# barry-mir/mixing-style-transfer

Measured on AMD Instinct MI355X. Metric: triplets/sec (10 s @ 44.1 kHz, 4-stem, bs=24), higher is better.
Workload: dtype f32

## Files before the change

### mixing-style-transfer_amd/csrc/encoder.hip

```cpp
#include "common.h"

#include <cmath>
#include <type_traits>
#include <vector>

namespace {

typedef float f32x4 __attribute__((ext_vector_type(4)));
constexpr int kConvThreads = 512;
constexpr int kConvWaves = 8;

struct FilmParams {
  const float* feats;
  const float *w0t, *b0, *w3t, *b3, *hwt, *hb;
  const float *s1, *t1, *s2, *t2;
  float* film;
  float2* aff1;
  float2* aff2;
  int Fd, H, nsub;
  float* h2;
  int B;
};

constexpr int kFilmCT = 8;
// ... 677 lines not shown
  int nsaddr[4] = {-1, -1, -1, -1};

  auto prefetch_setup = [&](int q, const RTile& t) __attribute__((always_inline)) {
    const int chunk = q % NCH;
    const float* src = p.in + (size_t)t.clip * p.in_clipstride + (size_t)t.band * p.in_bandoff + (size_t)(4 * chunk) * p.in_cstride;
    const float* wsrc = p.wfrag + ((size_t)t.band * NCH + chunk) * WBP;
    nrsrc = __builtin_amdgcn_make_buffer_rsrc(const_cast<float*>(src), 0, (unsigned)(4 * p.in_cstride) * 4u, 0x00020000);
    nwrsrc = __builtin_amdgcn_make_buffer_rsrc(const_cast<float*>(wsrc), 0, (unsigned)WBP * 4u, 0x00020000);
    if (chunk == 0) {
      const bool fold = t.kind == 2;
      const int row0 = (t.kind == 1 ? 4 : 0) - 3, col0 = 16 * t.blk - 3;
      const int rbase = max(row0, 0), cbase = max(col0, 0);
      nsoff = (unsigned)(rbase * p.in_cols + cbase) * 4u;
      int ln = lane;
      asm volatile("" : "+v"(ln));
#pragma unroll
      for (int j = 0; j < 4; ++j) {
        const int e = ln + 64 * j;
        const int r = fold ? e >> 4 : e / PC, c = fold ? e & 15 : e % PC;
        const bool in_patch = fold ? (r < R::FR && c < R::FC) : r < R::PR;
        const int rin = row0 + r, cin = col0 + c;
        const bool ok = t.valid && in_patch && rin >= 0 && rin < p.in_rows && cin >= 0 && cin < p.in_cols;
        nvoff[j] = ok ? (unsigned)((rin - rbase) * p.in_cols + (cin - cbase)) * 4u : 0x80000000u;
        nsaddr[j] = in_patch ? r * PC + c : -1;
      }
    }
  };
  auto prefetch_piece = [&](int i) __attribute__((always_inline)) {
    if (i < NPFK) {
      pf[i] = __builtin_bit_cast(float, __builtin_amdgcn_raw_buffer_load_b32(nrsrc, nvoff[i & 3], nsoff + (unsigned)((i >> 2) * p.in_cstride) * 4u, 0));
    } else if (i < NPIECE) {
      wreg[i - NPFK] = __builtin_bit_cast(f32x4, __builtin_amdgcn_raw_buffer_load_b128(nwrsrc, (unsigned)tid * 16u, (unsigned)(kConvThreads * (i - NPFK)) * 16u, 0));
    }
  };

  f32x4 acc[MT][NT];
  RTile cur{}, nxt{};
  nxt = decode(0);
  if (nq > 0) {
    prefetch_setup(0, nxt);
#pragma unroll
    for (int i = 0; i < NPIECE; ++i) prefetch_piece(i);
  }
#ifdef MST_TRACE
  long long trc[5] = {0, 0, 0, 0, 0};
  const long long trc_start = clock64();
#endif
  for (int q = 0; q < nq; ++q) {
    float* wb = wbuf + (q & 1) * WBP;
#ifdef MST_TRACE
    const long long tq0 = clock64();
#endif
#pragma unroll
    for (int i = 0; i < NWF; ++i) reinterpret_cast<f32x4*>(wb)[tid + kConvThreads * i] = wreg[i];
#pragma unroll
    for (int i = 0; i < NPFK; ++i)
      if (nsaddr[i & 3] >= 0) pbuf[(i >> 2) * CP + nsaddr[i & 3]] = pf[i];
#ifdef MST_TRACE
    asm volatile("s_waitcnt lgkmcnt(0)" ::: "memory");
    const long long tq1 = clock64();
#endif
    __syncthreads();
#ifdef MST_TRACE
    const long long tq2 = clock64();
    trc[0] += tq1 - tq0, trc[1] += tq2 - tq1, trc[4] += 1;
#endif
    cur = nxt;
    if ((q + 1) % NCH == 0) nxt = decode(q + 1);
    prefetch_setup(q + 1, nxt);
    const int chunk = q % NCH;
    if (chunk == 0) {
      ap = cur.kind == 2 ? ap_fold : ap_pair;
#pragma unroll
      for (int t = 0; t < MT; ++t)
#pragma unroll
        for (int n = 0; n < NT; ++n) acc[t][n] = f32x4{0.f, 0.f, 0.f, 0.f};
    }
    {
      float a[2][MT], b[2][NT];
#pragma unroll
      for (int t = 0; t < MT; ++t) a[0][t] = ap[t * PC];
#pragma unroll
      for (int n = 0; n < NT; ++n) b[0][n] = wb[n * 64 + lane];
      auto taps = [&](auto LO_, auto HI_, auto MASK_) __attribute__((always_inline)) {
        constexpr int LO = decltype(LO_)::value, HI = decltype(HI_)::value, MASK = decltype(MASK_)::value;
#pragma unroll
        for (int tap = LO; tap < HI; ++tap) {
          const int cu = tap & 1, nx = cu ^ 1;
          const int off = ((tap + 1) / 7) * PC + ((tap + 1) % 7);
#pragma unroll
          for (int i = 0; i < MT * NT; ++i) {
            const int t = i / NT, n = i % NT;
            if (!((MASK >> t) & 1)) acc[t][n] = __builtin_amdgcn_mfma_f32_16x16x4f32(a[cu][t], b[cu][n], acc[t][n], 0, 0, 0);
            if (tap + 1 < 49) {
              if (i < NT) b[nx][i] = wb[((tap + 1) * NT + i) * 64 + lane];
              else if (i < MT + NT) a[nx][i - NT] = ap[(i - NT) * PC + off];
            }
            if (i >= MT + NT && i - (MT + NT) < PPT) prefetch_piece(tap * PPT + (i - (MT + NT)));
            __builtin_amdgcn_sched_barrier(0);
          }
        }
      };
      using std::integral_constant;
      using I0 = integral_constant<int, 0>;
      using I7 = integral_constant<int, 7>;
      using I14 = integral_constant<int, 14>;
      using I21 = integral_constant<int, 21>;
      using I42 = integral_constant<int, 42>;
      using I49 = integral_constant<int, 49>;
      if (cur.kind == 0) {
        taps(I0{}, I7{}, integral_constant<int, 0b0111>{});
        taps(I7{}, I14{}, integral_constant<int, 0b0011>{});
        taps(I14{}, I21{}, integral_constant<int, 0b0001>{});
      } else {
        taps(I0{}, I21{}, I0{});
      }
      taps(I21{}, I42{}, I0{});
      if (cur.kind == 1) taps(I42{}, I49{}, integral_constant<int, 0b1000>{});
      else taps(I42{}, I49{}, I0{});
    }
#ifdef MST_TRACE
    trc[2] += clock64() - tq2;
#endif
    if (chunk == NCH - 1 && cur.valid) {
      const int j = lane & 15, g = lane >> 4;
      const float2* aff = p.aff + ((size_t)cur.clip * p.nsub + cur.band) * C::COUT;
      const int pr = cur.kind == 2 ? g >> 1 : cur.kind;
      const int pc = 4 * cur.blk + (cur.kind == 2 ? g & 1 : g);
#pragma unroll
      for (int n = 0; n < NT; ++n) {
        const int ch = n * 16 + j;
        const float2 ac = aff[ch];
        float m = 0.f;
#pragma unroll
        for (int t = 0; t < MT; ++t)
#pragma unroll
          for (int r = 0; r < 4; ++r) m = fmaxf(m, fmaf(acc[t][n][r], ac.x, ac.y));
        if (pc < p.out_cols)
          p.out[(((size_t)cur.clip * p.nsub + cur.band) * C::COUT + ch) * p.out_rows * p.out_cols + (size_t)pr * p.out_cols + pc] = m;
      }
    }
  }
#ifdef MST_TRACE
  if (lane == 0 && p.yraw) {
    float* o = p.yraw + (blockIdx.x * kConvWaves + wave) * 8;
    for (int i = 0; i < 5; ++i) o[i] = (float)trc[i];
    o[5] = (float)(clock64() - trc_start);
  }
#endif
}

template <int SUB>
constexpr size_t kConv1ResidentLds = (size_t)(2 * 49 * CC<1, SUB>::NT * 64 + kConvWaves * 8 * CC<1, SUB>::PR * CC<1, SUB>::PC) * sizeof(float);
template <int SUB, int MODE = 0, int LAY = 0>
__global__ __launch_bounds__(kConvThreads) void conv1_resident_kernel(const ConvParams p) {
  using C = CC<1, SUB>;
  constexpr int MT = C::MT, NT = C::NT, PR = C::PR, PC = C::PC;
  static_assert(C::RL == 64, "resident conv1 expects one loader row per instruction");
  static_assert(LAY == 0 || PR == 8, "the channel-minor loader maps lane bits 1..3 to the 8 patch rows");
  constexpr int WCH = 49 * NT * 64;
  constexpr int WBP = ConvGeom<1, SUB>::WBP;
  constexpr int CHS = PR * PC;
  constexpr int PATCH = 8 * CHS;
  constexpr int NPF = LAY == 0 ? 8 * PR : (PC + 3) / 4;
  extern __shared__ __attribute__((aligned(16))) float smem[];
  const int tid = threadIdx.x, lane = tid & 63;
  const int wave = __builtin_amdgcn_readfirstlane(tid >> 6);
  float* wres = smem;
  float* pbuf = smem + 2 * WCH + wave * PATCH;
  constexpr bool DYN = MODE == 0;
  constexpr int kTickets = 16;
  __shared__ unsigned tickets[kTickets];
#ifdef MST_TRACE
  long long trc[5] = {0, 0, 0, 0, 0};
  const long long trc_start = clock64();
#endif

  const int G = gridDim.x;
  const int wg = mst::xcd_remap(blockIdx.x, G);
  const int total_sets = (p.clip_major ? (p.B + p.clip_major - 1) / p.clip_major : 1) * p.nsub * p.sets_per_band;
  const int s_begin = (int)((long long)wg * total_sets / G), s_end = (int)((long long)(wg + 1) * total_sets / G);
  const int tpb = p.tiles_r * p.tiles_c;

  auto decode = [&](int s) __attribute__((always_inline)) {
    Tile t;
    int ti;
    if (p.clip_major) {
      const int ngrp = (p.B + p.clip_major - 1) / p.clip_major;
      const int gb = min(s / p.sets_per_band, ngrp * p.nsub - 1);
      const int idx = (s - gb * p.sets_per_band) * kConvWaves + wave;
      const int grp = gb / p.nsub, c0 = grp * p.clip_major;
      t.band = gb - grp * p.nsub;
      t.valid = (s < s_end) && idx < min(p.clip_major, p.B - c0) * tpb;
      const int cl = t.valid ? idx / tpb : 0;
      t.clip = c0 + cl;
      ti = t.valid ? idx - cl * tpb : 0;
    } else {
      t.band = min(s / p.sets_per_band, p.nsub - 1);
      const int idx = (s - t.band * p.sets_per_band) * kConvWaves + wave;
      t.valid = (s < s_end) && idx < p.B * tpb;
      t.clip = t.valid ? idx / tpb : 0;
      ti = t.valid ? idx - t.clip * tpb : 0;
    }
    t.tc = ti / p.tiles_r;
    t.tr = ti - t.tc * p.tiles_r;
    return t;
  };

  const int kq = lane >> 4, ai = lane & 15, ag = ai >> 2, areg = ai & 3;
  int abase[MT];
#pragma unroll
  for (int t = 0; t < MT; ++t) {
    const int e = 4 * t + areg, wv = e / C::WIN, pos = e % C::WIN;
    abase[t] = kq * CHS + (pos / 5) * PC + 5 * (C::WPG * ag + wv) + pos % 5;
  }

  typename std::conditional<LAY == 0, float, f32x4>::type pf[NPF];
  unsigned long long rowmask = 0;
  bool col_ok = false;
  int coff = 0, nrow0 = 0, nvalid = 0;
  const float* nsrc = p.in;
  bool nfast = false;
  __amdgpu_buffer_rsrc_t nrsrc = __builtin_amdgcn_make_buffer_rsrc(const_cast<float*>(p.in), 0, 0, 0x00020000);
  unsigned nsoff = 0, nvoff = 0;
  static_assert(WBP - WCH >= 4, "the chunk pitch leaves at least 16 zero bytes behind the weights");
  const float* const zero16 = p.wfrag + WCH;
  const int lr = (lane >> 1) & 7, lhalf = lane & 1, lfq = lane >> 4;
  const unsigned frame_bytes = (unsigned)p.cm_mels * 32u;
  auto prefetch_setup = [&](const Tile& t) __attribute__((always_inline)) {
    nrow0 = C::TROWS * t.tr - 3;
    nvalid = t.valid;
    rowmask = 0;
    if constexpr (LAY == 0) {
      const int col0 = C::TCOLS * t.tc - 3, cin = col0 + lane;
      nsrc = p.in + (size_t)t.clip * p.in_clipstride + (size_t)t.band * p.in_bandoff;
      col_ok = lane < PC && cin >= 0 && cin < p.in_cols;
      coff = min(max(cin, 0), p.in_cols - 1);
    } else {
      const int rin = nrow0 + lr, rc = min(max(rin, 0), p.in_rows - 1);
      nsrc = p.in + (size_t)t.clip * p.in_clipstride;
      col_ok = nvalid && rin == rc;
      coff = ((t.band * p.cm_overlap + rc) * 8 + 4 * lhalf) * 4;
      nrow0 = C::TCOLS * t.tc - 3 + lfq;
      if constexpr (DYN) {
        const int f0 = C::TCOLS * t.tc - 3;
        nfast = nvalid && f0 >= 0 && f0 + 4 * NPF + 3 < p.in_cols;
        nrsrc = __builtin_amdgcn_make_buffer_rsrc(const_cast<float*>(nsrc), 0, (unsigned)p.in_cols * frame_bytes, 0x00020000);
        nsoff = (unsigned)max(f0, 0) * frame_bytes;
        nvoff = col_ok ? (unsigned)coff + (unsigned)lfq * frame_bytes : 0x80000000u;
      }
    }
  };
  auto prefetch_piece = [&](int i) __attribute__((always_inline)) {
    if (i < NPF) {
      if constexpr (LAY == 0) {
        const int cc = i / PR, r = i % PR;
        const int rin = nrow0 + r;
        const int rc = min(max(rin, 0), p.in_rows - 1);
        if (nvalid && rin == rc) rowmask |= 1ull << i;
        const float* rowp = nsrc + (size_t)cc * p.in_cstride + (size_t)rc * p.in_cols;
        if constexpr (DYN) pf[i] = (nvalid && rin == rc && col_ok) ? rowp[coff] : *zero16;
        else pf[i] = rowp[coff];
      } else {
        const int fin = nrow0 + 4 * i, fc = min(max(fin, 0), p.in_cols - 1);
        if (col_ok && fin == fc) rowmask |= 1ull << i;
        if (DYN && nfast) {
          pf[i] = __builtin_bit_cast(f32x4, __builtin_amdgcn_raw_buffer_load_b128(nrsrc, nvoff, nsoff + (unsigned)(4 * i) * frame_bytes, 0));
        } else {
          const unsigned boff = (unsigned)fc * frame_bytes + (unsigned)coff;
          const char* src = reinterpret_cast<const char*>(nsrc) + boff;
          if constexpr (DYN) src = (col_ok && fin == fc) ? src : reinterpret_cast<const char*>(zero16);
          pf[i] = *reinterpret_cast<const f32x4*>(src);
        }
      }
    }
  };
  auto prefetch_step = [&](int ks) __attribute__((always_inline)) {
    if constexpr (LAY == 0) prefetch_piece(ks);
    else if (ks % 8 == 0) prefetch_piece(ks / 8);
  };

  f32x4 acc[MT][NT];
  double st[NT][2];
#pragma unroll
  for (int n = 0; n < NT; ++n) st[n][0] = st[n][1] = 0.0;
  int cur_band = -1;
  const int spb = p.sets_per_band;
  const int gb0 = s_begin / spb, nseg = s_end > s_begin ? (s_end - 1) / spb - gb0 + 1 : 0;
  int dseg = 0, dlo = 0, dhi = 0, dgb = 0, nxt_seg = 0;
  auto seg_range = [&](int k) __attribute__((always_inline)) {
    dgb = gb0 + k;
    const int cm = p.clip_major ? p.clip_major : p.B, grp = p.clip_major ? dgb / p.nsub : 0;
    dlo = max(s_begin - dgb * spb, 0) * kConvWaves;
    dhi = min((min(s_end, (dgb + 1) * spb) - dgb * spb) * kConvWaves, min(cm, p.B - grp * cm) * tpb);
  };
  unsigned tkv = 0;
  auto ticket_issue = [&]() __attribute__((always_inline)) {
    tkv = 0;
    if (dseg < nseg && lane == 0)
      tkv = __hip_atomic_fetch_add(&tickets[dseg % kTickets], 1u, __ATOMIC_RELAXED, __HIP_MEMORY_SCOPE_WORKGROUP);
  };
  auto ticket_take = [&]() __attribute__((always_inline)) {
    Tile t{};
    while (dseg < nseg) {
      const int idx = dlo + (int)__builtin_amdgcn_readfirstlane(tkv);
      if (idx < dhi) {
        const int grp = p.clip_major ? dgb / p.nsub : 0;
        const int cl = idx / tpb, ti = idx - cl * tpb;
        t.valid = 1;
        t.band = dgb - grp * p.nsub;
        t.clip = grp * p.clip_major + cl;
        t.tc = ti / p.tiles_r;
        t.tr = ti - t.tc * p.tiles_r;
        return t;
      }
      if (++dseg < nseg) seg_range(dseg);
      ticket_issue();
    }
    return t;
  };
  Tile cur{}, nxt{};
  if constexpr (DYN) {
    if (tid < kTickets) tickets[tid] = 0;
    __syncthreads();
    if (nseg > 0) seg_range(0);
    ticket_issue();
    nxt = ticket_take();
    nxt_seg = dseg;
  } else {
    nxt = decode(s_begin);
  }
  prefetch_setup(nxt);
#pragma unroll
  for (int i = 0; i < NPF; ++i) prefetch_piece(i);

  auto mask_piece = [&](int i) __attribute__((always_inline)) {
    if constexpr (LAY == 0) {
      pf[i] = (((rowmask >> i) & 1ull) && col_ok) ? pf[i] : 0.f;
    } else {
      const bool ok = (rowmask >> i) & 1ull;
#pragma unroll
      for (int k = 0; k < 4; ++k) pf[i][k] = ok ? pf[i][k] : 0.f;
    }
  };
  auto stage_ = [&](auto MASKED_) __attribute__((always_inline)) {
    constexpr bool MASKED = decltype(MASKED_)::value;
    if constexpr (LAY == 0) {
#pragma unroll
      for (int i = 0; i < NPF; ++i) {
        if (!MASKED) mask_piece(i);
        if (lane < PC) pbuf[i * PC + lane] = pf[i];
      }
    } else {
      float* pl = pbuf + (4 * lhalf) * CHS + lr * PC + lfq;
#pragma unroll
      for (int i = 0; i < NPF; ++i) {
        if (4 * i + 3 < PC || 4 * i + lfq < PC) {
          if (!MASKED) mask_piece(i);
#pragma unroll
          for (int k = 0; k < 4; ++k) pl[k * CHS + 4 * i] = pf[i][k];
        }
      }
    }
  };
  auto stage = [&]() __attribute__((always_inline)) { stage_(std::false_type{}); };
  auto tile_body = [&]() __attribute__((always_inline)) {
#ifdef MST_TRACE
    const long long tr0 = clock64();
#endif
#pragma unroll
    for (int t = 0; t < MT; ++t)
#pragma unroll
      for (int n = 0; n < NT; ++n) acc[t][n] = f32x4{0.f, 0.f, 0.f, 0.f};
    {
      float a[2][MT], b[2][NT];
#pragma unroll
      for (int t = 0; t < MT; ++t) a[0][t] = pbuf[abase[t]];
#pragma unroll
      for (int n = 0; n < NT; ++n) b[0][n] = wres[n * 64 + lane];
#pragma unroll
      for (int ks = 0; ks < 98; ++ks) {
        const int cu = ks & 1, nx = cu ^ 1;
        const int tap = (ks + 1) >> 1, ch = (ks + 1) & 1;
        const int off = ch * 4 * CHS + (tap / 7) * PC + (tap % 7);
#pragma unroll
        for (int i = 0; i < MT * NT; ++i) {
          const int t = i / NT, n = i % NT;
          acc[t][n] = __builtin_amdgcn_mfma_f32_16x16x4f32(a[cu][t], b[cu][n], acc[t][n], 0, 0, 0);
          if (ks + 1 < 98) {
            if (i < NT) b[nx][i] = wres[ch * WCH + (tap * NT + i) * 64 + lane];
            else if (i < MT + NT) a[nx][i - NT] = pbuf[abase[i - NT] + off];
          }
          if (i == MT + NT) prefetch_step(ks);
          __builtin_amdgcn_sched_barrier(0);
        }
      }
    }
#ifdef MST_TRACE
    const long long tr1 = clock64();
    trc[0] += tr1 - tr0, trc[4] += 1;
#endif
    if constexpr (MODE == 1) {
      const int j = lane & 15, g = lane >> 4;
      float* yb = p.yraw + ((((size_t)cur.clip * p.nsub + cur.band) * p.acc_tr + cur.tr) * p.acc_tc + cur.tc) *
                               (size_t)(NT * 64 * 4 * MT);
#pragma unroll
      for (int n = 0; n < NT; ++n) {
        const float b = p.bias[cur.band * C::COUT + n * 16 + j];
        f32x4* dst = reinterpret_cast<f32x4*>(yb) + (size_t)n * (64 * MT) + lane;
#pragma unroll
        for (int t = 0; t < MT; ++t) {
          f32x4 v = acc[t][n];
#pragma unroll
          for (int r = 0; r < 4; ++r) {
            v[r] += b;
            const int e = 4 * t + r, wv = e / C::WIN, pos = e % C::WIN;
            const int col = C::TCOLS * cur.tc + 5 * (C::WPG * g + wv) + pos % 5;
            if (col < p.raw_cols) st[n][0] += (double)v[r], st[n][1] += (double)v[r] * (double)v[r];
          }
          dst[64 * t] = v;
        }
      }
    } else
    {
      const int j = lane & 15, g = lane >> 4;
      const float2* aff = p.aff + ((size_t)cur.clip * p.nsub + cur.band) * C::COUT;
      float* orow = p.out + ((size_t)cur.clip * p.nsub + cur.band) * C::COUT * p.out_rows * p.out_cols +
                    (size_t)cur.tr * p.out_cols;
#pragma unroll
      for (int n = 0; n < NT; ++n) {
        const int ch = n * 16 + j;
        const float2 ac = aff[ch];
#pragma unroll
        for (int wv = 0; wv < C::WPG; ++wv) {
          const int pc = 4 * C::WPG * cur.tc + C::WPG * g + wv;
          if (SUB == 2 && p.pool_h == 1) {
#pragma unroll
            for (int hr = 0; hr < 2; ++hr) {
              float m = 0.f;
#pragma unroll
              for (int pos = 0; pos < 5; ++pos) {
                const int e = wv * C::WIN + 5 * hr + pos;
                m = fmaxf(m, fmaf(acc[e >> 2][n][e & 3], ac.x, ac.y));
              }
              if (pc < p.out_cols && 2 * cur.tr + hr < p.out_rows)
                orow[(size_t)ch * p.out_rows * p.out_cols + (size_t)(cur.tr + hr) * p.out_cols + pc] = m;
            }
          } else {
            float m = 0.f;
#pragma unroll
            for (int pos = 0; pos < C::WIN; ++pos) {
              const int e = wv * C::WIN + pos;
              m = fmaxf(m, fmaf(acc[e >> 2][n][e & 3], ac.x, ac.y));
            }
            if (pc < p.out_cols) orow[(size_t)ch * p.out_rows * p.out_cols + pc] = m;
          }
        }
      }
    }
#ifdef MST_TRACE
    trc[1] += clock64() - tr1;
#endif
  };
  f32x4 sav[MT][NT];
  float2 sav_ac[NT];
  Tile prev{};
#pragma unroll
  for (int t = 0; t < MT; ++t)
#pragma unroll
    for (int n = 0; n < NT; ++n) sav[t][n] = f32x4{0.f, 0.f, 0.f, 0.f};
#pragma unroll
  for (int n = 0; n < NT; ++n) sav_ac[n] = float2{0.f, 0.f};
  auto epi_part = [&](auto N_, auto WV_) __attribute__((always_inline)) {
    constexpr int n = decltype(N_)::value, wv = decltype(WV_)::value;
    const int j = lane & 15, g = lane >> 4;
    const int ch = n * 16 + j;
    float* orow = p.out + ((size_t)prev.clip * p.nsub + prev.band) * C::COUT * p.out_rows * p.out_cols + (size_t)prev.tr * p.out_cols;
    const float2 ac = sav_ac[n];
    const int pc = 4 * C::WPG * prev.tc + C::WPG * g + wv;
    if (SUB == 2 && p.pool_h == 1) {
#pragma unroll
      for (int hr = 0; hr < 2; ++hr) {
        float m = 0.f;
#pragma unroll
        for (int pos = 0; pos < 5; ++pos) {
          const int e = wv * C::WIN + 5 * hr + pos;
          m = fmaxf(m, fmaf(sav[e >> 2][n][e & 3], ac.x, ac.y));
        }
        if (prev.valid && pc < p.out_cols && 2 * prev.tr + hr < p.out_rows)
          orow[(size_t)ch * p.out_rows * p.out_cols + (size_t)(prev.tr + hr) * p.out_cols + pc] = m;
      }
    } else {
      float m = 0.f;
#pragma unroll
      for (int pos = 0; pos < C::WIN; ++pos) {
        const int e = wv * C::WIN + pos;
        m = fmaxf(m, fmaf(sav[e >> 2][n][e & 3], ac.x, ac.y));
      }
      if (prev.valid && pc < p.out_cols) orow[(size_t)ch * p.out_rows * p.out_cols + pc] = m;
    }
  };
  auto tile_dyn = [&]() __attribute__((always_inline)) {
#ifdef MST_TRACE
    const long long tr0 = clock64();
#endif
    float2 e_ac[NT];
    {
      const float2* aff = p.aff + ((size_t)cur.clip * p.nsub + cur.band) * C::COUT;
#pragma unroll
      for (int n = 0; n < NT; ++n) e_ac[n] = aff[n * 16 + (lane & 15)];
    }
    {
      constexpr int kEpi0 = 12;
      const bool skip_c = cur.tr == 0, skip_b = 2 * cur.tr + 2 >= p.in_rows;
      const int next_off = skip_b ? 0 : 5 * PC, next_w = skip_b ? 0 : 35 * NT * 64;
      float a[2][MT], b[2][NT];
#pragma unroll
      for (int t = 0; t < MT; ++t) a[0][t] = pbuf[abase[t] + 2 * PC];
#pragma unroll
      for (int n = 0; n < NT; ++n) b[0][n] = wres[(14 * NT + n) * 64 + lane];
      auto kstep = [&](auto S_) __attribute__((always_inline)) {
        constexpr int ks = decltype(S_)::value;
        constexpr int cu = ks & 1, nx = cu ^ 1;
        constexpr bool last = ks == 41 || ks == 69 || ks == 97;
        constexpr int s1 = ks + 1, l1 = s1 < 42 ? s1 : s1 < 70 ? s1 - 42 : s1 - 70;
        constexpr int row1 = (s1 < 42 ? 2 : s1 < 70 ? 5 : 0) + l1 / 14, tap1 = 7 * row1 + (l1 % 14) / 2, ch1 = l1 & 1;
        constexpr int off1 = ch1 * 4 * CHS + row1 * PC + (l1 % 14) / 2;
#pragma unroll
        for (int i = 0; i < MT * NT; ++i) {
          const int t = i / NT, n = i % NT;
          acc[t][n] = __builtin_amdgcn_mfma_f32_16x16x4f32(a[cu][t], b[cu][n], ks == 0 ? f32x4{0.f, 0.f, 0.f, 0.f} : acc[t][n], 0, 0, 0);
          if constexpr (!last) {
            if (i < NT) b[nx][i] = wres[ch1 * WCH + (tap1 * NT + i) * 64 + lane];
            else if (i < MT + NT) a[nx][i - NT] = pbuf[abase[i - NT] + off1];
          } else if constexpr (ks == 41) {
            if (i < NT) b[nx][i] = wres[next_w + i * 64 + lane];
            else if (i < MT + NT) a[nx][i - NT] = pbuf[abase[i - NT] + next_off];
          } else if constexpr (ks == 69) {
            if (i < NT) b[nx][i] = wres[i * 64 + lane];
            else if (i < MT + NT) a[nx][i - NT] = pbuf[abase[i - NT]];
          }
          if (i == MT + NT) {
            if constexpr (LAY == 0) {
              if constexpr (ks >= 8 && ks < 8 + NPF / 2) prefetch_piece(2 * (ks - 8)), prefetch_piece(2 * (ks - 8) + 1);
            } else {
              if constexpr (ks >= 8 && ks % 2 == 0 && ks / 2 - 4 < NPF) prefetch_piece(ks / 2 - 4);
            }
          }
          if (i == MT + NT + 1) {
            if constexpr (ks == 0) ticket_issue();
            if constexpr (ks == 6) {
              nxt = ticket_take();
              nxt_seg = dseg;
              prefetch_setup(nxt);
            }
            if constexpr (ks >= kEpi0 && ks < kEpi0 + 2 * NT * C::WPG && (ks - kEpi0) % 2 == 0)
              epi_part(std::integral_constant<int, (ks - kEpi0) / 2 / C::WPG>{}, std::integral_constant<int, (ks - kEpi0) / 2 % C::WPG>{});
          }
          __builtin_amdgcn_sched_barrier(0);
        }
      };
      static_assert(LAY == 0 ? 8 + NPF / 2 <= 42 : 2 * (NPF + 3) < 42, "the patch fetch must fit block A");
      static_for<42>([&](auto I) __attribute__((always_inline)) { kstep(std::integral_constant<int, decltype(I)::value>{}); });
      if (!skip_b) static_for<28>([&](auto I) __attribute__((always_inline)) { kstep(std::integral_constant<int, 42 + decltype(I)::value>{}); });
      if (!skip_c) static_for<28>([&](auto I) __attribute__((always_inline)) { kstep(std::integral_constant<int, 70 + decltype(I)::value>{}); });
    }
    {
      const float bz = wres[lane];
#pragma unroll
      for (int t = 0; t < MT; ++t)
#pragma unroll
        for (int n = 0; n < NT; ++n) sav[t][n] = __builtin_amdgcn_mfma_f32_16x16x4f32(0.f, bz, acc[t][n], 0, 0, 0);
    }
#pragma unroll
    for (int n = 0; n < NT; ++n) sav_ac[n] = e_ac[n];
    prev = cur;
#ifdef MST_TRACE
    trc[0] += clock64() - tr0, trc[4] += 1;
#endif
  };
  auto load_band = [&](int band) __attribute__((always_inline)) {
    for (int c = 0; c < 2; ++c) {
      const f32x4* src = reinterpret_cast<const f32x4*>(p.wfrag + ((size_t)band * 2 + c) * WBP);
      for (int k = tid; k < WCH / 4; k += kConvThreads) reinterpret_cast<f32x4*>(wres + c * WCH)[k] = src[k];
    }
  };
  if constexpr (DYN) {
    for (int k = 0; k < nseg; ++k) {
#ifdef MST_TRACE
      const long long tb0 = clock64();
#endif
      __syncthreads();
      load_band((gb0 + k) % p.nsub);
      if (tid == 0) tickets[(k + kTickets - 1) % kTickets] = 0;
      __syncthreads();
#ifdef MST_TRACE
      trc[3] += clock64() - tb0;
#endif
      while (nxt.valid && nxt_seg == k) {
#ifdef MST_TRACE
        const long long ts0 = clock64();
#endif
        cur = nxt;
#ifdef MST_TRACE
        asm volatile("s_waitcnt vmcnt(0)" ::: "memory");
        const long long ts1 = clock64();
        trc[1] += ts1 - ts0;
#endif
        stage_(std::true_type{});
#ifdef MST_TRACE
        asm volatile("s_waitcnt lgkmcnt(0)" ::: "memory");
        trc[2] += clock64() - ts1;
#endif
        tile_dyn();
      }
    }
    {
      static_for<NT * C::WPG>([&](auto I) __attribute__((always_inline)) {
        constexpr int q = decltype(I)::value;
        epi_part(std::integral_constant<int, q / C::WPG>{}, std::integral_constant<int, q % C::WPG>{});
      });
    }
#ifdef MST_TRACE
    if (lane == 0 && p.yraw) {
      float* o = p.yraw + (blockIdx.x * kConvWaves + wave) * 8;
      for (int i = 0; i < 5; ++i) o[i] = (float)trc[i];
      o[5] = (float)(clock64() - trc_start);
    }
#endif
  } else {
  for (int s = s_begin; s < s_end; ++s) {
    cur = nxt;
    if (cur.band != cur_band) {
      if (MODE == 1 && cur_band >= 0) flush_stats<NT, C::COUT>(st, p.stats, cur_band, lane);
      __syncthreads();
      load_band(cur.band);
      __syncthreads();
      cur_band = cur.band;
    }
    stage();
    nxt = decode(s + 1);
    prefetch_setup(nxt);
    if (!cur.valid) {
#pragma unroll
      for (int i = 0; i < NPF; ++i) prefetch_piece(i);
      continue;
    }
    tile_body();
  }
  }
  if (MODE == 1 && cur_band >= 0) flush_stats<NT, C::COUT>(st, p.stats, cur_band, lane);
}

__global__ __launch_bounds__(256) void absmax_kernel(const float* __restrict__ x, long long n_per_clip, unsigned* out) {
  const float* base = x + (size_t)blockIdx.y * n_per_clip;
  float m = 0.f;
  const long long n4 = n_per_clip >> 2;
  const float4* b4 = reinterpret_cast<const float4*>(base);
  const bool al = (reinterpret_cast<uintptr_t>(base) & 15) == 0;
  if (al) {
    for (long long i = (long long)blockIdx.x * 256 + threadIdx.x; i < n4; i += (long long)gridDim.x * 256) {
      const float4 v = b4[i];
      m = fmaxf(fmaxf(m, fmaxf(fabsf(v.x), fabsf(v.y))), fmaxf(fabsf(v.z), fabsf(v.w)));
    }
    for (long long i = (n4 << 2) + (long long)blockIdx.x * 256 + threadIdx.x; i < n_per_clip; i += (long long)gridDim.x * 256)
      m = fmaxf(m, fabsf(base[i]));
  } else {
    for (long long i = (long long)blockIdx.x * 256 + threadIdx.x; i < n_per_clip; i += (long long)gridDim.x * 256)
      m = fmaxf(m, fabsf(base[i]));
  }
  m = mst::wave_max(m);
  if ((threadIdx.x & 63) == 0) atomicMax(out + blockIdx.y, __float_as_uint(m));
}

__global__ __launch_bounds__(64) void f16_scale_kernel(const float2* __restrict__ aff1, const float* __restrict__ w1norm,
                                                        const unsigned* __restrict__ xmax_bits, float* scale, int nsub,
                                                        const float* __restrict__ bias = nullptr, float gain = 1.0f) {
  const int clip = blockIdx.x / nsub, band = blockIdx.x % nsub, c = threadIdx.x & 31;
  const float xmax = __uint_as_float(xmax_bits[clip]);
  const float2 a = aff1[((size_t)clip * nsub + band) * 32 + c];
  float bound = fmaf(fabsf(a.x), fmaf(w1norm[band * 32 + c], xmax, bias ? fabsf(bias[band * 32 + c]) : 0.f), fabsf(a.y)) * gain;
  bound = mst::wave_max(bound);
  if (threadIdx.x == 0) {
    int k = 0;
    if (bound > 0.f && bound < INFINITY) {
      int ex;
      (void)frexpf(bound, &ex);
      k = max(-60, min(60, 14 - ex));
    } else if (!(bound < INFINITY)) {
      k = -60;
    }
    scale[(size_t)blockIdx.x * 2] = ldexpf(1.0f, k);
    scale[(size_t)blockIdx.x * 2 + 1] = ldexpf(1.0f, -k);
  }
}

typedef _Float16 h16x8 __attribute__((ext_vector_type(8)));
__device__ __forceinline__ _Float16 to_f16_sat(float v) {
  return (_Float16)(__builtin_isfinite(v) ? fminf(fmaxf(v, -65504.f), 65504.f) : v);
}
__host__ inline int f16_weight_exponent(float maxabs) {
  if (!(maxabs > 0.f) || !(maxabs < INFINITY)) return 10;
  int ex;
  (void)frexpf(maxabs, &ex);
  return std::max(-100, std::min(100, 14 - ex));
}
constexpr int kF16Steps = 13;

template <int SUB>
constexpr size_t kConv1F16Lds = (size_t)(kF16Steps * CC<1, SUB>::NT * 2 * 64 + kConvWaves * 2 * CC<1, SUB>::PR * CC<1, SUB>::PC) * 16;
template <int SUB, int TERMS, int MODE = 0, int LAY = 0>
__global__ __launch_bounds__(kConvThreads) void conv1_f16x3_kernel(const ConvParams p, const h16x8* __restrict__ wfrag16,
                                                                  _Float16* __restrict__ out_hi, _Float16* __restrict__ out_lo) {
  using C = CC<1, SUB>;
  constexpr int MT = C::MT, NT = C::NT, PR = C::PR, PC = C::PC;
  static_assert(C::RL == 64, "one loader row per instruction");
  static_assert(LAY == 0 || (LAY == 2 && PR == 8), "the channel-minor loader maps lane bits 0..2 to the 8 patch rows");
  constexpr int WVEC = kF16Steps * NT * 2 * 64;
// ... 2175 lines not shown
  float* ptrs[] = {e->w1frag, e->w2frag, e->s1, e->t1, e->s2, e->t2, e->w0t, e->b0, e->w3t, e->b3, e->hwt,
                   e->hb, e->att0frag, e->att0_b, e->att2_w, e->projfrag, e->proj_b, e->c1b, e->bn1w, e->bn1b, e->c2b,
                   e->bn2w, e->bn2b, e->w2dfrag, e->att2_b, e->f16_wsc1e, e->f16_wsc2e, e->w2norm_e};
  for (float* q : ptrs) (void)hipFree(q);
  (void)hipFree(e->w1frag16), (void)hipFree(e->w1frag16e);
  (void)hipFree(e->w1norm), (void)hipFree(e->f16_winv1), (void)hipFree(e->f16_winv2);
  (void)hipFree(e->w2frag16);
  (void)hipFree(e->w2dfrag16);
  (void)hipFree(e->f16_wsc1), (void)hipFree(e->f16_wsc2), (void)hipFree(e->f16_wsc2d), (void)hipFree(e->f16_winv2d);
  (void)hipFree(e->w2norm);
  delete e;
}

int mst_encoder_set_precision(mst_encoder* e, int conv1_f16x3) {
  MST_REQUIRE(e, "mst_encoder_set_precision: NULL encoder");
  MST_REQUIRE(conv1_f16x3 == 0 || (conv1_f16x3 >= 1 && conv1_f16x3 <= 3 && (e->sub == 2 || (e->sub == 1 && e->cfg.split_size % 2 == 0))),
              "mst_encoder_set_precision: the f16 modes (1, 2, 3) need 2-row conv1 tiles (20-mel sub-bands, or an even split_size below 20)");
  e->conv1_f16x3 = conv1_f16x3;
  return MST_OK;
}

int mst_encoder_set_train_precision(mst_encoder* e, int f16_operands) {
  MST_REQUIRE(e, "mst_encoder_set_train_precision: NULL encoder");
  MST_REQUIRE(f16_operands == 0 || ((f16_operands == 1 || f16_operands == 2) && (e->sub == 2 || e->cfg.split_size % 2 == 0)),
              "mst_encoder_set_train_precision: modes 1 (f16 operands) and 2 (split precision) need 2-row conv1 tiles (20-mel sub-bands, or an even split_size below 20)");
  if (f16_operands && !e->w2dfrag16) {
    const int ns = e->cfg.n_subbands;
    bool ok = hipMalloc(&e->w2dfrag16, (size_t)ns * 8 * kF16Steps * 2 * 2 * 64 * 8 * sizeof(_Float16)) == hipSuccess;
    ok = ok && hipMalloc(&e->f16_wsc1, (size_t)ns * 32 * 4) == hipSuccess && hipMalloc(&e->f16_wsc2, (size_t)ns * 64 * 4) == hipSuccess;
    ok = ok && hipMalloc(&e->f16_wsc2d, (size_t)ns * 32 * 4) == hipSuccess && hipMalloc(&e->f16_winv2d, (size_t)ns * 32 * 4) == hipSuccess;
    ok = ok && hipMalloc(&e->w2norm, (size_t)ns * 64 * 4) == hipSuccess;
    if (!ok) return mst::fail(MST_ENOMEM, "mst_encoder_set_train_precision: out of device memory");
  }
  e->train_f16 = f16_operands;
  return MST_OK;
}

size_t mst_encoder_workspace_bytes(const mst_encoder* e, int B, int frames) {
  if (!e || B <= 0 || frames < 20) return 0;
  return ws_layout(e, B, frames).total;
}

static bool conv1_resident_geometry(const mst_encoder* e) {
  return (e->sub == 2 || (e->sub == 1 && e->cfg.split_size % 2 == 0)) && !getenv("MST_CONV1_CHUNKED");
}

int mst_encoder_layout_supported(const mst_encoder* e, int layout) {
  if (!e) return 0;
  if (layout == MST_LOGMEL_REF) return 1;
  if (e->sub > 2) return 0;
  if (layout == MST_LOGMEL_CM32) return e->conv1_f16x3 == 0 && conv1_resident_geometry(e);
  if (layout == MST_LOGMEL_CM16) return e->conv1_f16x3 != 0;
  return 0;
}

int mst_encoder_forward(const mst_encoder* e, const float* logmel, int frames, const float* feats, int B, float* emb,
                        const mst_encoder_taps* taps, void* workspace, size_t workspace_bytes, void* stream) {
  mst_logmel_in in{};
  in.layout = MST_LOGMEL_REF, in.data = logmel;
  return mst_encoder_forward_in(e, &in, frames, feats, B, emb, taps, workspace, workspace_bytes, stream);
}

int mst_encoder_forward_in(const mst_encoder* e, const mst_logmel_in* lin, int frames, const float* feats, int B, float* emb,
                           const mst_encoder_taps* taps, void* workspace, size_t workspace_bytes, void* stream) {
  MST_REQUIRE(e && lin && lin->data && feats && emb, "mst_encoder_forward: NULL argument");
  const int lay = lin->layout;
  if (const int rc = check_logmel_in("mst_encoder_forward", lin, mst_encoder_layout_supported(e, lay), e->conv1_f16x3,
                                     e->conv1_f16x3 != 3, e->conv1_f16x3 >= 2))
    return rc;
  const float* logmel = static_cast<const float*>(lin->data);
  MST_REQUIRE(B > 0 && frames >= 20, "mst_encoder_forward: need B>0 and frames>=20 (B=%d frames=%d)", B, frames);
  const WsLayout L = ws_layout(e, B, frames);
  MST_REQUIRE(L.W2 >= 1, "mst_encoder_forward: clip too short for two pooling stages (frames=%d)", frames);
  if (!workspace || workspace_bytes < L.total)
    return mst::fail(MST_ENOMEM, "mst_encoder_forward: workspace %zu B < required %zu B", workspace_bytes, L.total);
  hipStream_t st = reinterpret_cast<hipStream_t>(stream);
  char* ws = reinterpret_cast<char*>(workspace);
  const int ns = e->cfg.n_subbands;
  float* film = (taps && taps->film) ? taps->film : reinterpret_cast<float*>(ws + L.film);
  float* pool1 = (taps && taps->pool1) ? taps->pool1 : reinterpret_cast<float*>(ws + L.pool1);
  float* pool_in = (taps && taps->pool_in) ? taps->pool_in : reinterpret_cast<float*>(ws + L.pool_in);
  float2* aff1 = reinterpret_cast<float2*>(ws + L.aff1);
  float2* aff2 = reinterpret_cast<float2*>(ws + L.aff2);
  auto mark = [&](int i) {
    if (taps && taps->events[i]) (void)hipEventRecord(reinterpret_cast<hipEvent_t>(taps->events[i]), st);
  };
  mark(0);
  MST_HIP_CHECK(launch_film(film_params(e, feats, film, aff1, aff2, reinterpret_cast<float*>(ws + L.film_h2), B), st));
  mark(1);
  const int grid = e->num_cus;
  const dim3 blk(kConvThreads);
  {
    ConvParams cp{};
    cp.in = logmel, cp.wfrag = e->w1frag, cp.aff = aff1, cp.out = pool1, cp.B = B, cp.nsub = ns;
    conv1_input_geometry(cp, e, frames);
    cp.in_lo = lin->lo, cp.cm_mels = e->cfg.n_mels, cp.cm_overlap = e->cfg.overlap;
    cp.out_rows = e->H1, cp.out_cols = L.W1;
    cp.tiles_r = e->H1;
    cp.tiles_c = e->sub == 2 ? (L.W1 + 7) / 8 : (L.W1 + 15) / 16;
    const bool resident = e->sub <= 2 && !e->conv1_f16x3 && conv1_resident_geometry(e);
    if (e->sub == 1 && (e->conv1_f16x3 || resident)) {
      cp.pool_h = 1;
      cp.tiles_r = e->cfg.split_size / 2;
      cp.tiles_c = (L.W1 + 7) / 8;
    }
    cp.sets_per_band = sets_per_band(B, cp.tiles_r, cp.tiles_c);
    const int g = std::min(grid, ns * cp.sets_per_band);
    hipError_t err;
    if (e->sub > 2) {
      MST_REQUIRE(lay == MST_LOGMEL_REF && e->conv1_f16x3 == 0, "mst_encoder_forward: split_size=%d runs in the reference layout, fp32 only", e->cfg.split_size);
      err = mst::launch_lds<conv1_generic_kernel>(dim3((L.W1 + kGenCols - 1) / kGenCols, B * ns), dim3(256),
                                                  conv1_generic_lds(e->cfg.split_size), st, cp, e->sub);
    } else if (e->conv1_f16x3) {
      const bool both = e->conv1_f16x3 >= 2;
      cp.f16_winv = e->f16_winv1;
      if (both && !(taps && taps->pool1)) cp.out = nullptr;
      if (both) {
        const unsigned* xmax = lin->absmax;
        float* fsc = reinterpret_cast<float*>(ws + L.f16scale);
        if (!xmax) {
          unsigned* xm = reinterpret_cast<unsigned*>(ws + L.xmax);
          MST_HIP_CHECK(hipMemsetAsync(xm, 0, (size_t)B * sizeof(unsigned), st));
          const long long npc = (long long)8 * e->cfg.n_mels * frames;
          hipLaunchKernelGGL(absmax_kernel, dim3(64, B), dim3(256), 0, st, logmel, npc, xm);
          xmax = xm;
        }
        hipLaunchKernelGGL(f16_scale_kernel, dim3(B * ns), dim3(64), 0, st, aff1, e->w1norm, xmax, fsc, ns);
        cp.f16_scale = fsc;
      }
      const h16x8* wf = reinterpret_cast<const h16x8*>(e->w1frag16);
      _Float16* oh = both ? reinterpret_cast<_Float16*>(ws + L.pool1_h16) : nullptr;
      _Float16* ol = e->conv1_f16x3 == 2 ? reinterpret_cast<_Float16*>(ws + L.pool1_l16) : nullptr;
      if (lay == MST_LOGMEL_CM16) {
        const h16x8* wfe = reinterpret_cast<const h16x8*>(e->w1frag16e);
        if (e->conv1_f16x3 == 3) {
          cp.sets_per_band = sets_per_band(B, cp.tiles_r, cp.tiles_c, kF16eWaves<1>);
          const int g1 = std::min(grid, ns * cp.sets_per_band);
          err = mst::launch_lds<conv1_f16e_kernel<1>>(dim3(g1), dim3(kF16eWaves<1> * 64), kConv1F16eLds<1>, st, cp, wfe, oh, ol);
        }
        else err = mst::launch_lds<conv1_f16e_kernel<3>>(dim3(g), blk, kConv1F16eLds<3>, st, cp, wfe, oh, ol);
      } else if (e->conv1_f16x3 == 3) err = mst::launch_lds<conv1_f16x3_kernel<2, 1>>(dim3(g), blk, kConv1F16Lds<2>, st, cp, wf, oh, ol);
      else err = mst::launch_lds<conv1_f16x3_kernel<2, 3>>(dim3(g), blk, kConv1F16Lds<2>, st, cp, wf, oh, ol);
    } else if (resident) {
      if (!getenv("MST_CONV1_BAND_MAJOR")) {
        const char* env = getenv("MST_CONV1_CLIP_GROUP");
        cp.clip_major = std::max(1, std::min(B, env ? atoi(env) : 1));
        cp.sets_per_band = sets_per_band(cp.clip_major, cp.tiles_r, cp.tiles_c);
      }
      const int g = std::min(grid, (cp.clip_major ? (B + cp.clip_major - 1) / cp.clip_major : 1) * ns * cp.sets_per_band);
#ifdef MST_TRACE
      static ConvTrace trace;
      trace_attach(trace, cp);
#endif
      if (lay == MST_LOGMEL_CM32) err = mst::launch_lds<conv1_resident_kernel<2, 0, 1>>(dim3(g), blk, kConv1ResidentLds<2>, st, cp);
      else err = mst::launch_lds<conv1_resident_kernel<2>>(dim3(g), blk, kConv1ResidentLds<2>, st, cp);
#ifdef MST_TRACE
      trace_dump(trace, g, false);
#endif
    } else {
      err = e->sub == 2 ? launch_conv<1, 2>(cp, g, st) : launch_conv<1, 1>(cp, g, st);
    }
    if (err != hipSuccess) return mst::fail(MST_EHIP, "conv1 launch failed: %s", hipGetErrorString(err));
  }
  mark(2);
  {
    ConvParams cp{};
    cp.in = pool1, cp.wfrag = e->w2frag, cp.aff = aff2, cp.out = pool_in, cp.B = B, cp.nsub = ns;
    conv2_input_geometry(cp, e, L.W1);
    cp.out_rows = e->FD, cp.out_cols = L.W2;
    cp.tiles_r = (e->FD + 1) / 2;
    cp.tiles_c = (L.W2 + 1) / 2;
    cp.sets_per_band = sets_per_band(B, cp.tiles_r, cp.tiles_c);
    const int g = std::min(grid, ns * cp.sets_per_band);
    hipError_t err;
    if (e->conv1_f16x3 >= 2) {
      cp.f16_scale = reinterpret_cast<const float*>(ws + L.f16scale);
      cp.f16_winv = e->f16_winv2;
      const h16x8* ih = reinterpret_cast<const h16x8*>(ws + L.pool1_h16);
      const h16x8* il = reinterpret_cast<const h16x8*>(ws + L.pool1_l16);
      const h16x8* wf = reinterpret_cast<const h16x8*>(e->w2frag16);
      if (e->conv1_f16x3 == 3) err = mst::launch_lds<conv2_f16x3_kernel<1>>(dim3(g), blk, kConv2F16Lds, st, cp, ih, il, wf);
      else err = mst::launch_lds<conv2_f16x3_kernel<3>>(dim3(g), blk, kConv2F16Lds, st, cp, ih, il, wf);
    } else {
#ifdef MST_TRACE
      static ConvTrace trace;
      trace_attach(trace, cp);
#endif
      const char* tiles_env = getenv("MST_CONV2_TILES");
      if (e->FD == 2 && e->H1 == 10 && !(tiles_env && !strcmp(tiles_env, "8x8"))) {
        const int rem = L.W2 % 4;
        cp.rt_blocks = L.W2 / 4 + (rem == 3);
        cp.rt_fold = rem == 1 || rem == 2;
        cp.rt_pair_sets = (B * cp.rt_blocks + 3) / 4;
        cp.sets_per_band = cp.rt_pair_sets + (B * cp.rt_fold + kConvWaves - 1) / kConvWaves;
        err = mst::launch_lds<conv2_rows_kernel>(dim3(std::min(grid, ns * cp.sets_per_band)), blk, RowTiles::kLds, st, cp);
      } else {
        err = launch_conv<2, 2>(cp, g, st);
      }
#ifdef MST_TRACE
      trace_dump(trace, g, true);
#endif
    }
    if (err != hipSuccess) return mst::fail(MST_EHIP, "conv2 launch failed: %s", hipGetErrorString(err));
  }
  mark(3);
  if (const int rc = launch_head(e, L, ws, pool_in, emb, B, st, taps ? taps->events[4] : nullptr)) return rc;
  mark(5);
  return MST_OK;
}

namespace {
struct TrainLayout {
  WsLayout base;
  size_t y1, y2, stats1, stats2, bn1, bn2, dfilm_acc, dw_acc, total;
  size_t t_pool1_h16, t_pool1_l16, t_f16scale, t_xmax, t_bscale, t_dyg1, t_dyg2, t_ys1, t_ys2;
  int tr1, tc1, tr2, tc2;
};
TrainLayout train_layout(const mst_encoder* e, int B, int frames) {
  TrainLayout T{};
  T.base = ws_layout(e, B, frames);
  const int ns = e->cfg.n_subbands;
  const bool two_row = e->sub == 2 || train_fwd16(e);
  const int tcols1 = two_row ? 40 : 80;
  T.tr1 = two_row ? e->cfg.split_size / 2 : e->H1, T.tc1 = (frames + tcols1 - 1) / tcols1;
  T.tr2 = (e->H1 + 7) / 8, T.tc2 = (T.base.W1 + 7) / 8;
  size_t o = T.base.total;
  auto take = [&](size_t bytes) {
    const size_t at = o;
    o += mst::align_up(bytes, 256);
    return at;
  };
  const size_t ybytes = e->train_f16 == 1 ? 2 : 4;
  T.y1 = take((size_t)B * ns * T.tr1 * T.tc1 * 2 * 64 * 20 * ybytes);
  T.y2 = take((size_t)B * ns * T.tr2 * T.tc2 * 4 * 64 * 16 * ybytes);
  T.stats1 = take((size_t)(ns * 32 * 2 + 1) * sizeof(mst::DetAcc));
  T.stats2 = take((size_t)(ns * 64 * 2 + 1) * sizeof(mst::DetAcc));
  T.bn1 = take((size_t)ns * 32 * 8);
  T.bn2 = take((size_t)ns * 64 * 8);
  T.dfilm_acc = take((size_t)B * ns * 192 * sizeof(mst::DetAcc));
  T.dw_acc = take((size_t)ns * 64 * 1568 * sizeof(mst::DetAcc));
  const size_t f = train_fwd16(e) ? 1 : 0, fb = train_bwd16(e) ? 1 : 0;
  T.t_pool1_h16 = take(f * (size_t)B * ns * 32 * e->H1 * T.base.W1 * 2);
  T.t_pool1_l16 = take((e->train_f16 == 2 ? 1 : 0) * (size_t)B * ns * 32 * e->H1 * T.base.W1 * 2);
  T.t_f16scale = take(f * (size_t)B * ns * 2 * 4);
  T.t_xmax = take(f * (size_t)B * 4);
  T.t_ys1 = take((e->train_f16 == 1 ? 1 : 0) * (size_t)ns * 2 * 4);
  T.t_ys2 = take((e->train_f16 == 1 ? 1 : 0) * (size_t)ns * 2 * 4);
  T.t_bscale = take(fb * 16);
  const size_t cgs = (size_t)((B + 7) / 8);
  const size_t hl = e->train_f16 == 2 ? 2 : 1;
  T.t_dyg1 = take(fb * hl * (size_t)ns * cgs * T.tr1 * T.tc1 * 2 * 20 * 64 * 16);
  T.t_dyg2 = take(fb * hl * (size_t)ns * cgs * T.tr2 * T.tc2 * 4 * 16 * 64 * 16);
  T.total = o;
  return T;
}
}

size_t mst_encoder_train_workspace_bytes(const mst_encoder* e, int B, int frames) {
  if (!e || B <= 0 || frames < 20 || e->sub > 2) return 0;
  return train_layout(e, B, frames).total;
}

int mst_encoder_train_stats_buffer(const mst_encoder* e, int layer, int B, int frames, size_t* offset_bytes, size_t* n_int64) {
  MST_REQUIRE(e && offset_bytes && n_int64 && (layer == 1 || layer == 2) && B > 0 && frames >= 20,
              "mst_encoder_train_stats_buffer: bad arguments");
  const TrainLayout T = train_layout(e, B, frames);
  *offset_bytes = layer == 1 ? T.stats1 : T.stats2;
  *n_int64 = ((size_t)e->cfg.n_subbands * (layer == 1 ? 32 : 64) * 2 + 1) * (sizeof(mst::DetAcc) / 8);
  return MST_OK;
}

int mst_encoder_train_scale_buffer(const mst_encoder* e, int B, int frames, size_t* offset_bytes) {
  MST_REQUIRE(e && offset_bytes && B > 0 && frames >= 20, "mst_encoder_train_scale_buffer: bad arguments");
  MST_REQUIRE(train_bwd16(e), "mst_encoder_train_scale_buffer: the fp32 training mode has no internal loss scale");
  *offset_bytes = train_layout(e, B, frames).t_bscale + 2 * sizeof(float);
  return MST_OK;
}

int mst_encoder_train_layout_supported(const mst_encoder* e, int layout) {
  if (!e) return 0;
  if (layout == MST_LOGMEL_REF) return 1;
  if (layout == MST_LOGMEL_CM16) return train_fwd16(e) ? 1 : 0;
  return 0;
}

int mst_encoder_forward_train(const mst_encoder* e, const float* logmel, int frames, const float* feats, int B, float* emb,
                              const mst_encoder_train_taps* taps, void* workspace, size_t workspace_bytes, void* stream) {
  mst_logmel_in in{};
  in.layout = MST_LOGMEL_REF, in.data = logmel;
  return mst_encoder_forward_train_in(e, &in, frames, feats, B, emb, taps, workspace, workspace_bytes, stream);
}

int mst_encoder_forward_train_in(const mst_encoder* e, const mst_logmel_in* lin, int frames, const float* feats, int B, float* emb,
                                 const mst_encoder_train_taps* taps, void* workspace, size_t workspace_bytes, void* stream) {
  MST_REQUIRE(e && e->sub <= 2, "mst_encoder_forward_train: the training kernels cover first-pool heights 1 and 2 (split_size < 30)");
  MST_REQUIRE(e && lin && lin->data && (feats || (taps && taps->film_in)), "mst_encoder_forward_train: NULL argument");
  const int lay = lin->layout;
  if (const int rc = check_logmel_in("mst_encoder_forward_train", lin, mst_encoder_train_layout_supported(e, lay), e->train_f16,
                                     e->train_f16 != 1, false))
    return rc;
  const float* logmel = static_cast<const float*>(lin->data);
  MST_REQUIRE(B > 0 && frames >= 20, "mst_encoder_forward_train: need B>0 and frames>=20 (B=%d frames=%d)", B, frames);
  const TrainLayout T = train_layout(e, B, frames);
  const WsLayout& L = T.base;
  MST_REQUIRE(L.W2 >= 1, "mst_encoder_forward_train: clip too short for two pooling stages (frames=%d)", frames);
  if (!workspace || workspace_bytes < T.total)
    return mst::fail(MST_ENOMEM, "mst_encoder_forward_train: workspace %zu B < required %zu B", workspace_bytes, T.total);
  hipStream_t st = reinterpret_cast<hipStream_t>(stream);
// ... 581 lines not shown
```

Baseline: 2841.

## Row-sort conv1 MFMA tiles to skip padded-row MMAs at band edges

Adds a ROWS variant of the resident conv1 kernel that remaps patch elements so each MFMA A-tile covers a single output row. At the top and bottom tile edges, where some kernel rows fall in zero padding, whole MFMA tiles can then be skipped through compile-time masks. The epilogue goes through a slot permutation to undo the remap. The variant is on by default for sub=2 and trades extra code variants (more instruction-cache pressure) for fewer MFMAs on edge tiles only.

New measurement: 2861 (median of 6 runs). No clear change (+0.7%).

```diff
diff --git a/mixing-style-transfer_amd/csrc/encoder.hip b/mixing-style-transfer_amd/csrc/encoder.hip
--- a/mixing-style-transfer_amd/csrc/encoder.hip
+++ b/mixing-style-transfer_amd/csrc/encoder.hip
@@ -853,11 +853,18 @@
 
 template <int SUB>
 constexpr size_t kConv1ResidentLds = (size_t)(2 * 49 * CC<1, SUB>::NT * 64 + kConvWaves * 8 * CC<1, SUB>::PR * CC<1, SUB>::PC) * sizeof(float);
-template <int SUB, int MODE = 0, int LAY = 0>
+template <bool ROWS>
+__host__ __device__ constexpr int conv1_slot(int e) {
+  if (!ROWS) return e;
+  const int row = e % 10 / 5, q = 5 * (e / 10) + e % 5;
+  return q < 8 ? 4 * (2 * row + q / 4) + q % 4 : 16 + 2 * row + (q - 8);
+}
+template <int SUB, int MODE = 0, int LAY = 0, bool ROWS = false>
 __global__ __launch_bounds__(kConvThreads) void conv1_resident_kernel(const ConvParams p) {
   using C = CC<1, SUB>;
   constexpr int MT = C::MT, NT = C::NT, PR = C::PR, PC = C::PC;
   static_assert(C::RL == 64, "resident conv1 expects one loader row per instruction");
+  static_assert(!ROWS || (SUB == 2 && MODE == 0 && MT == 5), "the row-sorted map is the eval forward's, on 2 x 40 tiles");
   static_assert(LAY == 0 || PR == 8, "the channel-minor loader maps lane bits 1..3 to the 8 patch rows");
   constexpr int WCH = 49 * NT * 64;
   constexpr int WBP = ConvGeom<1, SUB>::WBP;
@@ -912,8 +919,13 @@
   int abase[MT];
 #pragma unroll
   for (int t = 0; t < MT; ++t) {
-    const int e = 4 * t + areg, wv = e / C::WIN, pos = e % C::WIN;
-    abase[t] = kq * CHS + (pos / 5) * PC + 5 * (C::WPG * ag + wv) + pos % 5;
+    if constexpr (ROWS) {
+      const int row = t < 4 ? t >> 1 : areg >> 1, q = t < 4 ? 4 * (t & 1) + areg : 8 + (areg & 1);
+      abase[t] = kq * CHS + row * PC + 10 * ag + q;
+    } else {
+      const int e = 4 * t + areg, wv = e / C::WIN, pos = e % C::WIN;
+      abase[t] = kq * CHS + (pos / 5) * PC + 5 * (C::WPG * ag + wv) + pos % 5;
+    }
   }
 
   typename std::conditional<LAY == 0, float, f32x4>::type pf[NPF];
@@ -1186,7 +1198,7 @@
 #pragma unroll
         for (int pos = 0; pos < 5; ++pos) {
           const int e = wv * C::WIN + 5 * hr + pos;
-          m = fmaxf(m, fmaf(sav[e >> 2][n][e & 3], ac.x, ac.y));
+          m = fmaxf(m, fmaf(sav[conv1_slot<ROWS>(e) >> 2][n][conv1_slot<ROWS>(e) & 3], ac.x, ac.y));
         }
         if (prev.valid && pc < p.out_cols && 2 * prev.tr + hr < p.out_rows)
           orow[(size_t)ch * p.out_rows * p.out_cols + (size_t)(prev.tr + hr) * p.out_cols + pc] = m;
@@ -1196,7 +1208,7 @@
 #pragma unroll
       for (int pos = 0; pos < C::WIN; ++pos) {
         const int e = wv * C::WIN + pos;
-        m = fmaxf(m, fmaf(sav[e >> 2][n][e & 3], ac.x, ac.y));
+        m = fmaxf(m, fmaf(sav[conv1_slot<ROWS>(e) >> 2][n][conv1_slot<ROWS>(e) & 3], ac.x, ac.y));
       }
       if (prev.valid && pc < p.out_cols) orow[(size_t)ch * p.out_rows * p.out_cols + pc] = m;
     }
@@ -1220,8 +1232,8 @@
       for (int t = 0; t < MT; ++t) a[0][t] = pbuf[abase[t] + 2 * PC];
 #pragma unroll
       for (int n = 0; n < NT; ++n) b[0][n] = wres[(14 * NT + n) * 64 + lane];
-      auto kstep = [&](auto S_) __attribute__((always_inline)) {
-        constexpr int ks = decltype(S_)::value;
+      auto kstep = [&](auto S_, auto MASK_) __attribute__((always_inline)) {
+        constexpr int ks = decltype(S_)::value, MASK = decltype(MASK_)::value;
         constexpr int cu = ks & 1, nx = cu ^ 1;
         constexpr bool last = ks == 41 || ks == 69 || ks == 97;
         constexpr int s1 = ks + 1, l1 = s1 < 42 ? s1 : s1 < 70 ? s1 - 42 : s1 - 70;
@@ -1230,7 +1242,8 @@
 #pragma unroll
         for (int i = 0; i < MT * NT; ++i) {
           const int t = i / NT, n = i % NT;
-          acc[t][n] = __builtin_amdgcn_mfma_f32_16x16x4f32(a[cu][t], b[cu][n], ks == 0 ? f32x4{0.f, 0.f, 0.f, 0.f} : acc[t][n], 0, 0, 0);
+          if (ks == 0 || !((MASK >> t) & 1))
+            acc[t][n] = __builtin_amdgcn_mfma_f32_16x16x4f32(a[cu][t], b[cu][n], ks == 0 ? f32x4{0.f, 0.f, 0.f, 0.f} : acc[t][n], 0, 0, 0);
           if constexpr (!last) {
             if (i < NT) b[nx][i] = wres[ch1 * WCH + (tap1 * NT + i) * 64 + lane];
             else if (i < MT + NT) a[nx][i - NT] = pbuf[abase[i - NT] + off1];
@@ -1262,9 +1275,39 @@
         }
       };
       static_assert(LAY == 0 ? 8 + NPF / 2 <= 42 : 2 * (NPF + 3) < 42, "the patch fetch must fit block A");
-      static_for<42>([&](auto I) __attribute__((always_inline)) { kstep(std::integral_constant<int, decltype(I)::value>{}); });
-      if (!skip_b) static_for<28>([&](auto I) __attribute__((always_inline)) { kstep(std::integral_constant<int, 42 + decltype(I)::value>{}); });
-      if (!skip_c) static_for<28>([&](auto I) __attribute__((always_inline)) { kstep(std::integral_constant<int, 70 + decltype(I)::value>{}); });
+      auto ksteps = [&](auto LO_, auto N_, auto MASK_) __attribute__((always_inline)) {
+        static_for<decltype(N_)::value>([&](auto I) __attribute__((always_inline)) {
+          kstep(std::integral_constant<int, decltype(LO_)::value + decltype(I)::value>{}, MASK_);
+        });
+      };
+      using std::integral_constant;
+      using All = integral_constant<int, 0>;
+      using I14 = integral_constant<int, 14>;
+      using I28 = integral_constant<int, 28>;
+      if constexpr (!ROWS) {
+        ksteps(All{}, integral_constant<int, 42>{}, All{});
+        if (!skip_b) ksteps(integral_constant<int, 42>{}, I28{}, All{});
+        if (!skip_c) ksteps(integral_constant<int, 70>{}, I28{}, All{});
+      } else {
+        using Up = integral_constant<int, 0b00011>;
+        using Lo = integral_constant<int, 0b01100>;
+        const bool lo6 = 2 * cur.tr + 4 >= p.in_rows;
+        if (skip_c) ksteps(All{}, I14{}, Up{});
+        else ksteps(All{}, I14{}, All{});
+        ksteps(I14{}, I14{}, All{});
+        if (skip_b) ksteps(I28{}, I14{}, Lo{});
+        else ksteps(I28{}, I14{}, All{});
+        if (!skip_b) {
+          ksteps(integral_constant<int, 42>{}, I14{}, All{});
+          if (lo6) ksteps(integral_constant<int, 56>{}, I14{}, Lo{});
+          else ksteps(integral_constant<int, 56>{}, I14{}, All{});
+        }
+        if (!skip_c) {
+          if (cur.tr == 1) ksteps(integral_constant<int, 70>{}, I14{}, Up{});
+          else ksteps(integral_constant<int, 70>{}, I14{}, All{});
+          ksteps(integral_constant<int, 84>{}, I14{}, All{});
+        }
+      }
     }
     {
       const float bz = wres[lane];
@@ -3746,8 +3789,15 @@
       static ConvTrace trace;
       trace_attach(trace, cp);
 #endif
-      if (lay == MST_LOGMEL_CM32) err = mst::launch_lds<conv1_resident_kernel<2, 0, 1>>(dim3(g), blk, kConv1ResidentLds<2>, st, cp);
-      else err = mst::launch_lds<conv1_resident_kernel<2>>(dim3(g), blk, kConv1ResidentLds<2>, st, cp);
+      const char* tiles_env = getenv("MST_CONV1_TILES");
+      const bool rows = e->sub == 2 && !(tiles_env && !strcmp(tiles_env, "mixed"));
+      if (lay == MST_LOGMEL_CM32) {
+        if (rows) err = mst::launch_lds<conv1_resident_kernel<2, 0, 1, true>>(dim3(g), blk, kConv1ResidentLds<2>, st, cp);
+        else err = mst::launch_lds<conv1_resident_kernel<2, 0, 1>>(dim3(g), blk, kConv1ResidentLds<2>, st, cp);
+      } else {
+        if (rows) err = mst::launch_lds<conv1_resident_kernel<2, 0, 0, true>>(dim3(g), blk, kConv1ResidentLds<2>, st, cp);
+        else err = mst::launch_lds<conv1_resident_kernel<2>>(dim3(g), blk, kConv1ResidentLds<2>, st, cp);
+      }
 #ifdef MST_TRACE
       trace_dump(trace, g, false);
 #endif
```
